# logicxin/SwiftMPI

Hardware: AMD Instinct MI355X
Metric: SGNS trained words/sec at 1/8 GPUs; sparse push/pull HBM GB/s vs peak (higher is better)
Workload: dtype f32 table, block-fp intermediates (int32 mantissas/row exponent), f64 accumulate; 1 GPU; word2vec CBOW-NS (the reference's 'SGNS' app) text8-shaped corpus 17005207 tokens, vocab 253628, dim 300, window 5, negative 5, sample 1e-05, minibatch 5000 lines of 1000 tokens, table in one HBM shard; global_batch=5000, parallelism=1 GPU, one HBM shard, batches_per_epoch=5

## Files before the change

### swiftmpi_amd/csrc/swps_w2v.hip

```cpp
#include <algorithm>
#include <cstdlib>
#include <cstdio>

#include "swps_w2v_ctx.h"

using namespace swps;

namespace {

__global__ void k_vid_keys(const int32_t *__restrict__ K, uint64_t n, const uint64_t *__restrict__ vkeys,
                           uint64_t *__restrict__ out) {
  uint64_t i = (uint64_t)blockIdx.x * blockDim.x + threadIdx.x;
  if (i < n) out[i] = vkeys[K[i]];
}

__global__ void k_stamp_rows(const uint32_t *__restrict__ rows, uint64_t n, uint32_t cap, uint32_t stamp,
                             uint32_t *__restrict__ mark) {
  const uint64_t i = (uint64_t)blockIdx.x * blockDim.x + threadIdx.x;
  if (i < n && rows[i] < cap) mark[rows[i]] = stamp;
}
__global__ void k_flag_rows(const uint32_t *__restrict__ rows, uint64_t n, uint32_t cap, uint32_t stamp,
                            const uint32_t *__restrict__ mark, uint8_t *__restrict__ flags) {
  const uint64_t i = (uint64_t)blockIdx.x * blockDim.x + threadIdx.x;
  if (i < n) flags[i] = rows[i] >= cap || mark[rows[i]] == stamp;
// ... 7 lines not shown
  if (!t || !cfg || !out) return fail(SWPS_E_CFG, "null argument");
  *out = nullptr;
  if (t->cfg.layout != SWPS_LAYOUT_W2V) return fail(SWPS_E_CFG, "table layout must be SWPS_LAYOUT_W2V");
  SWPS_TRY(check_app_table(t));
  SWPS_HIP(hipSetDevice(t->cfg.device));
  swps_w2v *w = new swps_w2v();
  w->t = t;
  w->cfg = *cfg;
  w->D = t->cfg.dim;
  w->W = cfg->window;
  w->N = cfg->negative;
  w->f64 = t->cfg.dtype == SWPS_F64;
  w->s = t->stream;
  w->timer.on = cfg->profile != 0;
  if (const char *e = getenv("SWPS_XCD_ORDER")) w->xcd_order = atoi(e) != 0;
  if (const char *e = getenv("SWPS_PUSH_T")) w->push_t = atoi(e) != 0;
  if (const char *e = getenv("SWPS_FUSED_PUSH")) w->fused_push = atoi(e) != 0;
  if (const char *e = getenv("SWPS_COMBINE")) w->combine = atoi(e);
  if (const char *e = getenv("SWPS_COMBINE_MIN")) w->combine_min = strtoull(e, nullptr, 10);
  if (const char *e = getenv("SWPS_FULL_LINES")) w->full_lines = atoi(e) != 0;
  if (const char *e = getenv("SWPS_SPLIT_PUSH")) w->split_push = atoi(e);
  if (const char *e = getenv("SWPS_SPLIT_GRADS")) w->split_grads = atoi(e) != 0;
  if (const char *e = getenv("SWPS_PUSH_GRID")) w->push_grid = (uint32_t)std::max(0, atoi(e));
  if (const char *e = getenv("SWPS_MULTI_SORT")) w->multi_sort = atoi(e);
  if (const char *e = getenv("SWPS_MULTI_CHUNK")) w->multi_chunk = (uint32_t)std::min(128, std::max(0, atoi(e)));
  if (const char *e = getenv("SWPS_MULTI_SORT_MIN")) w->multi_sort_min = strtoull(e, nullptr, 10);
  if (const char *e = getenv("SWPS_ROW_PAD")) w->row_pad = atoi(e) != 0;
  if (const char *e = getenv("SWPS_UNI_INDEX")) w->uni_index = atoi(e) != 0;
  if (const char *e = getenv("SWPS_SEG4")) w->seg4 = atoi(e) != 0;
  if (const char *e = getenv("SWPS_TOK_LOCAL")) w->tok_local = atoi(e) != 0;
  if (const char *e = getenv("SWPS_ITEM_HEADS")) w->item_heads = atoi(e) != 0;
  if (const char *e = getenv("SWPS_CACHE_PAD")) w->cache_pad = atoi(e) != 0;
  if (const char *e = getenv("SWPS_OVERLAP")) w->overlap = atoi(e);
  if (const char *e = getenv("SWPS_REC_GENERIC")) w->rec_generic = atoi(e) != 0;
  if (const char *e = getenv("SWPS_GATHER_GRID")) w->gather_grid = std::max(64, atoi(e));
  if (const char *e = getenv("SWPS_PUSH_WPE")) w->push_wpe = atoi(e);
  if (const char *e = getenv("SWPS_PUSH_UNR8")) w->push_unr = atoi(e) ? 8 : 4;
  int rc = check_cfg(w);
  if (!rc && hipHostMalloc((void **)&w->h_small, 64) != hipSuccess) rc = fail(SWPS_E_OOM, "pinned alloc");
  if (!rc) rc = w->d_rows_touched.ensure(16);
  if (!rc && hipMemset(w->d_rows_touched.p, 0, 16) != hipSuccess) rc = fail(SWPS_E_HIP, "memset");
  if (!rc) rc = w->d_gstats.ensure(32);
  if (!rc && hipMemset(w->d_gstats.p, 0, 32) != hipSuccess) rc = fail(SWPS_E_HIP, "memset");
  if (!rc) rc = upload_lcg_constants();
  if (rc) {
    if (w->h_small) (void)hipHostFree(w->h_small);
    delete w;
    return rc;
  }
  *out = w;
  return SWPS_OK;
}

int swps_w2v_destroy(swps_w2v *w) {
  if (!w) return SWPS_OK;
  (void)hipSetDevice(w->t->cfg.device);
  (void)hipStreamSynchronize(w->s);
  if (w->s_prep) {
    (void)hipStreamSynchronize(w->s_prep);
    (void)hipStreamDestroy(w->s_prep);
  }
  if (w->s_side) {
    (void)hipStreamSynchronize(w->s_side);
    (void)hipStreamDestroy(w->s_side);
  }
  if (w->ev_learn) (void)hipEventDestroy(w->ev_learn);
  if (w->ev_prep) (void)hipEventDestroy(w->ev_prep);
  if (w->ev_fwd) (void)hipEventDestroy(w->ev_fwd);
  if (w->ev_half) (void)hipEventDestroy(w->ev_half);
  if (w->ev_gat) (void)hipEventDestroy(w->ev_gat);
  if (w->h_small) (void)hipHostFree(w->h_small);
  delete w->drv;
  delete w;
  (void)hipGetLastError();
  return SWPS_OK;
}

int swps_w2v_load_text(swps_w2v *w, const char *path) {
  if (!w->cfg.minibatch_vocab && !w->cfg.host_ingest) {
    FILE *f = fopen(path, "rb");
    if (!f) return fail(SWPS_E_IO, std::string("no such file or directory: ") + path);
    std::vector<char> text;
    char chunk[1 << 16];
    size_t k;
    while ((k = fread(chunk, 1, sizeof(chunk), f)) > 0) text.insert(text.end(), chunk, chunk + k);
    fclose(f);
    if (!memchr(text.data(), 0, text.size())) {
      SWPS_HIP(hipSetDevice(w->t->cfg.device));
      DevMem d_keys;
      uint64_t nt = 0;
      std::vector<int64_t> off;
      SWPS_TRY(tokenize_gpu(w, text, d_keys, nt, off));
      std::vector<char>().swap(text);
      SWPS_TRY(ingest_gpu(w, d_keys, nt, std::move(off)));
      SWPS_TRY(schedule_gpu(w));
      return upload_corpus(w);
    }
  }
  FILE *f = fopen(path, "rb");
  if (!f) return fail(SWPS_E_IO, std::string("no such file or directory: ") + path);
// ... 123 lines not shown
}

int swps_w2v_train_batches(swps_w2v *w, uint64_t count) {
  if (!w->inited) return fail(SWPS_E_STATE, "call swps_w2v_init first");
  if (w->drv) {
    SWPS_HIP(hipSetDevice(w->t->cfg.device));
    return w->drv->steps(count);
  }
  if (w->sharded) return fail(SWPS_E_STATE, "sharded context: drive it with request / serve_pull / step / serve_push");
  SWPS_HIP(hipSetDevice(w->t->cfg.device));
  const bool ov = w->overlap > 0 || (w->overlap < 0 && w->max_tok <= kOverlapTok);
  if (ov && count > 1 && !w->cfg.minibatch_vocab && w->trace.size() >= w->trace_cap && !w->pb.valid)
    return train_overlapped(w, count);
  for (uint64_t i = 0; i < count; i++) SWPS_TRY(learn_step(w));
  return SWPS_OK;
}

int swps_w2v_train_epochs(swps_w2v *w, int32_t niters) {
  if (w->drv) {
    if (w->drv->spe && w->drv->cursor % w->drv->spe) return fail(SWPS_E_STATE, "not at an epoch boundary");
    SWPS_TRY(swps_w2v_train_batches(w, (uint64_t)niters * w->drv->spe));
    return swps_w2v_sync(w);
  }
  if (w->cursor % std::max<size_t>(1, w->batches.size()) != 0) return fail(SWPS_E_STATE, "not at an epoch boundary");
  SWPS_TRY(swps_w2v_train_batches(w, (uint64_t)niters * w->batches.size()));
  return swps_w2v_sync(w);
}

int swps_w2v_sync(swps_w2v *w) {
  SWPS_HIP(hipSetDevice(w->t->cfg.device));
  if (w->drv) SWPS_TRY(w->drv->sync());
  SWPS_HIP(hipStreamSynchronize(w->s));
  if (w->ss) SWPS_HIP(hipStreamSynchronize(w->ss));
  w->timer.resolve();
  return SWPS_OK;
}

int swps_w2v_stats(swps_w2v *w, uint64_t *o) {
  o[0] = w->st_batches;
  o[1] = w->st_kept;
  o[2] = w->st_words;
  o[3] = w->st_pairs;
  o[4] = w->lstate;
  o[5] = w->fstate;
  o[6] = w->st_pulled;
  o[7] = w->st_pushed;
  uint64_t rt[2] = {0, 0};
  SWPS_HIP(hipStreamSynchronize(w->s));
  SWPS_HIP(hipMemcpy(rt, w->d_rows_touched.p, 16, hipMemcpyDeviceToHost));
  o[8] = rt[0];
  o[9] = rt[1];
  return SWPS_OK;
}

int swps_w2v_gather_stats(swps_w2v *w, uint64_t *out2) {
  SWPS_HIP(hipStreamSynchronize(w->s));
  SWPS_HIP(hipMemcpy(out2, w->d_gstats.p, 16, hipMemcpyDeviceToHost));
  return SWPS_OK;
}

int swps_w2v_sum_stats(swps_w2v *w, uint64_t *out8) {
  SWPS_HIP(hipStreamSynchronize(w->s));
  SWPS_HIP(hipMemcpy(out8, w->d_gstats.p, 32, hipMemcpyDeviceToHost));
  out8[4] = w->st_fused;
  out8[5] = w->st_sums;
  out8[6] = w->st_fused_g;
// ... 420 lines not shown
  if (head[1] != w2v_corpus_fp(w) || head[2] != V || head[3] != ((uint64_t)w->D | ((uint64_t)es << 32)))
    return fail(SWPS_E_CFG, "snapshot was taken on a different corpus");
  if (head[4] != w->t->snap_sum)
    return fail(SWPS_E_STATE, "the table was not restored from the table snapshot saved with this worker state "
                              "(swps_restore <prefix>.table of the same save first)");
  std::vector<char> ch(V * w->D * es), cv(ch.size());
  SWPS_TRY(f.get(ch.data(), ch.size()));
  SWPS_TRY(f.get(cv.data(), cv.size()));
  SWPS_TRY(f.finish_read());
  if (!w->sharded) {
    DevMem dk;
    SWPS_TRY(upload(dk, w->vocab_keys, w->s));
    SWPS_TRY(table_lookup(w->t, dk.as<uint64_t>(), V, w->d_vid_row.as<uint32_t>(), w->s));
    if (table_check_error(w->t, w->s) != SWPS_OK)
      return fail(SWPS_E_STATE, "the table lacks the worker's vocab rows: swps_restore its table snapshot first");
  }
  if (!ch.empty()) {
    SWPS_HIP(hipMemcpy2D(w->d_cache_h.p, (size_t)w->cs * es, ch.data(), w->D * es, w->D * es, V,
                         hipMemcpyHostToDevice));
    SWPS_HIP(hipMemcpy2D(w->d_cache_v.p, (size_t)w->cs * es, cv.data(), w->D * es, w->D * es, V,
                         hipMemcpyHostToDevice));
  }
  SWPS_HIP(hipMemcpy(w->d_rows_touched.p, st + 9, 16, hipMemcpyHostToDevice));
  w->cursor = st[0];
  w->lstate = st[1];
  w->fstate = st[2];
  w->st_batches = st[3];
  w->st_kept = st[4];
  w->st_words = st[5];
  w->st_pairs = st[6];
  w->st_pulled = st[7];
  w->st_pushed = st[8];
  w->pb = swps_w2v::Prepped();
  const uint64_t nb = std::max<uint64_t>(1, w->batches.size());
  if (w->cursor % nb != 0) SWPS_TRY(plan_epoch(w));
  if (w->drv) {
    if (w->cursor % nb != 0) return fail(SWPS_E_STATE, "library-driven sharded state not at an epoch boundary");
    w->drv->cursor = w->cursor / nb * w->drv->spe;
    if (w->drv->ops.set_serve_stream) SWPS_TRY(w->drv->ops.set_serve_stream(w, w->drv->S));
  }
  w->inited = true;
  return SWPS_OK;
}

}
```

### swiftmpi_amd/csrc/swps_w2v_ctx.h

```cpp
#pragma once
#include <limits>
#include <memory>
#include <utility>
#include <vector>

#include "swps_internal.h"

namespace swps {

constexpr int32_t kTabRow = 0x40000000;
constexpr int kUShift = 10;

constexpr int kBfpMaxD = 512;
inline int bfp_ld(int D, int RB) { return (D + RB * D / 4 + 1 + 31) / 32 * 32; }
inline int bfp_shape(int D) {
  const int nch = D / 256, rem = D % 256;
  if (rem == 0) return 10 * nch;
  if (rem <= 128) return 10 * nch + (rem + 63) / 64;
  return 10 * (nch + 1);
}

enum { KT_KEEP = 0, KT_FWD, KT_SORT, KT_GATHER, KT_PUSH, KT_PULL, KT_REC, KT_N };

inline int row_ld(int D, size_t es, bool pad = true) {
// ... 142 lines not shown
  std::vector<uint64_t> icounts;
  std::vector<int32_t> init_order;
  DevMem d_vkeys, d_init_order, d_serve_rows, d_push_rows;
  DevMem d_mark;
  const uint32_t *pull_rows = nullptr;
  struct Parts {
    const void *vals[2] = {nullptr, nullptr};
    const uint32_t *pos[2] = {nullptr, nullptr};
    uint64_t n[2] = {0, 0};
  } parts;
  uint32_t mark_stamp = 0;
  hipStream_t ss = nullptr;
  int64_t slot = -1;
  struct SlotRows {
    DevMem rows, sorted;
    uint64_t n = 0;
    bool sorted_valid = false;
  };
  std::vector<std::unique_ptr<SlotRows>> slot_rows;
  std::vector<uint32_t> plan_P;
  std::vector<int32_t> allUK;
  std::vector<uint64_t> bstarts;
  std::vector<int32_t> bcnt_tok;
  uint64_t gather_end = 0;
  DevMem d_bstarts, d_UK, d_bcnt_tok, d_tw;
  std::vector<uint2> alias;
  DevMem d_alias;
  struct Prepped {
    bool valid = false, records = false, sorted = false, msorted = false;
    uint64_t bi = 0, P = 0, nt = 0, HOFF = 0, M = 0, max_items = 0;
    uint32_t U = 0;
  } pb;
  static constexpr int kPrepBufs = 15;
  DevMem alt[kPrepBufs];
  bool alt_local_ready = false;
  int overlap = -1;
  hipStream_t s_prep = nullptr;
  hipEvent_t ev_learn = nullptr, ev_prep = nullptr;
  hipEvent_t fwd_event = nullptr;
  DevMem *prep_set[kPrepBufs] = {&d_pos_tok, &d_rec,  &d_pkeys, &d_pvals, &d_pkeys_s, &d_pvals_s, &d_tmp,
                                 &d_seg,     &d_icnt, &d_ioff,  &d_desc,  &d_lead,    &d_multi, &d_krow, &d_local};
  uint64_t st_batches = 0, st_kept = 0, st_words = 0, st_pairs = 0, st_pulled = 0, st_pushed = 0;
  uint64_t st_sums = 0, st_fused = 0, st_fused_g = 0, st_split = 0;
  uint64_t trace_cap = 0;
  std::vector<int64_t> trace;
  Timer timer;
};

namespace swps {

constexpr uint32_t kChunk = 128;
inline uint32_t multi_chunk(const swps_w2v *w, uint64_t) { return w->multi_chunk ? w->multi_chunk : kChunk; }
constexpr uint64_t kOverlapTok = 1000000;

int check_cfg(swps_w2v *w);
int ingest(swps_w2v *w, const std::vector<uint64_t> &tok_keys, std::vector<int64_t> &&line_off);
void unigram_starts(const uint64_t *keys, const int32_t *counts, size_t V, uint64_t T, std::vector<uint64_t> &starts);
void build_schedule(swps_w2v *w);
int build_schedule_mb(swps_w2v *w);
int tokenize_gpu(swps_w2v *w, const std::vector<char> &text, DevMem &d_keys, uint64_t &nt,
                 std::vector<int64_t> &line_off);
int token_keys_gpu(swps_w2v *w, const uint32_t *word_ids, uint64_t ntok, const uint64_t *word_keys, uint64_t nwords,
                   DevMem &d_keys);
int ingest_gpu(swps_w2v *w, DevMem &d_keys, uint64_t nt, std::vector<int64_t> &&line_off);
int schedule_gpu(swps_w2v *w);
int upload_corpus(swps_w2v *w);

int upload_lcg_constants();
int plan_epoch(swps_w2v *w);
int prep_batch(swps_w2v *w);

int learn_step(swps_w2v *w, const void *d_vals = nullptr, void *d_grads = nullptr);
int train_overlapped(swps_w2v *w, uint64_t count);
int pull_all(swps_w2v *w);
int rand_init_gpu(swps_w2v *w);
int set_hv(swps_w2v *w, const double *hv);
int install_init(swps_w2v *w, const void *d_vals);

}
```

### swiftmpi_amd/csrc/swps_w2v_ingest.hip

```cpp
#include <algorithm>
#include <cmath>
#include <map>
#include <unordered_map>
#include <unordered_set>

#include "swps_scan.h"
#include "swps_sort.h"
#include "swps_w2v_ctx.h"

using namespace swps;

namespace {

__global__ void k_build_unigram(const uint64_t *__restrict__ starts, uint32_t V, uint64_t T, int32_t *__restrict__ table) {
  uint64_t a = (uint64_t)blockIdx.x * blockDim.x + threadIdx.x;
  uint64_t stride = (uint64_t)gridDim.x * blockDim.x;
  for (; a < T; a += stride) {
    uint32_t lo = 0, hi = V;
    while (hi - lo > 1) {
      uint32_t mid = (lo + hi) >> 1;
      if (starts[mid] <= a)
        lo = mid;
      else
        hi = mid;
// ... 710 lines not shown
  SWPS_TRY(lix.ensure((nb + 1) * 4));
  k_text_flags<<<nblk(nb + 1), 256, 0, s>>>(d_text.as<char>(), nb, st.as<uint32_t>(), nlf.as<uint32_t>());
  SWPS_HIP(hipGetLastError());
  SWPS_TRY(exclusive_scan(st.as<const uint32_t>(), tix.as<uint32_t>(), nb + 1, tmp, s));
  SWPS_TRY(exclusive_scan(nlf.as<const uint32_t>(), lix.as<uint32_t>(), nb + 1, tmp, s));
  uint32_t tot[2];
  SWPS_HIP(hipMemcpyAsync(&tot[0], tix.as<uint32_t>() + nb, 4, hipMemcpyDeviceToHost, s));
  SWPS_HIP(hipMemcpyAsync(&tot[1], lix.as<uint32_t>() + nb, 4, hipMemcpyDeviceToHost, s));
  SWPS_HIP(hipStreamSynchronize(s));
  nt = tot[0];
  const uint64_t nnl = tot[1];
  const uint64_t nlines = nnl + ((nb && text[nb - 1] != '\n') ? 1 : 0);
  SWPS_TRY(tstart.ensure(std::max<uint64_t>(nt, 1) * 8));
  SWPS_TRY(d_off.ensure((nlines + 2) * 8));
  SWPS_HIP(hipMemsetAsync(d_off.p, 0, 8, s));
  if (nb)
    k_text_index<<<nblk(nb), 256, 0, s>>>(d_text.as<char>(), nb, st.as<uint32_t>(), tix.as<uint32_t>(),
                                           lix.as<uint32_t>(), tstart.as<uint64_t>(), d_off.as<int64_t>());
  SWPS_HIP(hipGetLastError());
  SWPS_TRY(d_keys.ensure(std::max<uint64_t>(nt, 1) * 8));
  if (nt)
    k_text_keys<<<nblk(nt), 256, 0, s>>>(d_text.as<char>(), nb, tstart.as<uint64_t>(), nt,
                                          w->cfg.key_mode == SWPS_KEY_ATOI, d_keys.as<uint64_t>());
  SWPS_HIP(hipGetLastError());
  line_off.assign(nlines + 1, 0);
  if (nnl) SWPS_HIP(hipMemcpyAsync(line_off.data(), d_off.p, (nnl + 1) * 8, hipMemcpyDeviceToHost, s));
  SWPS_HIP(hipStreamSynchronize(s));
  line_off[nlines] = (int64_t)nt;
  return SWPS_OK;
}

int upload_corpus(swps_w2v *w) {
  hipStream_t s = w->s;
  const uint64_t V = w->vocab_keys.size();
  if (!w->tok_on_device) {
    SWPS_TRY(upload(w->d_tok, w->tok, s));
    SWPS_TRY(upload(w->d_tok_line, w->tok_line, s));
    SWPS_TRY(upload(w->d_K, w->allK, s));
  }
  SWPS_TRY(upload(w->d_line_off, w->line_off, s));
  SWPS_TRY(tok_fingerprint(w));
  std::vector<int64_t> btok;
  for (auto &b : w->batches) btok.push_back(w->line_off[b.l0]);
  btok.push_back(w->line_off[w->batches.back().l1]);
  SWPS_TRY(upload(w->d_btok, btok, s));
  std::vector<float> ran(V);
  for (uint64_t i = 0; i < V; i++) {
    float freq = float(w->counts[i]) / (float)w->train_words;
    ran[i] = (float)(1 - std::sqrt((double)(w->cfg.sample / freq)));
  }
  SWPS_TRY(upload(w->d_ran, ran, s));
  std::vector<float> ex(1000);
  for (int i = 0; i < 1000; i++) {
    float x = (i / (float)1000 * 2 - 1) * 6;
    float e = (float)std::exp((double)x);
    ex[i] = e / (e + 1);
  }
  SWPS_TRY(upload(w->d_exptab, ex, s));
  if (w->cfg.sampler == SWPS_SAMPLER_ALIAS) {
    if (!w->cfg.minibatch_vocab) {
      w->alias.clear();
      build_alias(w->counts.data(), V, w->alias);
    }
    SWPS_TRY(upload(w->d_alias, w->alias, s));
  }
  if (w->cfg.minibatch_vocab) {
    SWPS_TRY(upload(w->d_bstarts, w->bstarts, s));
    SWPS_TRY(upload(w->d_UK, w->allUK, s));
    SWPS_TRY(upload(w->d_bcnt_tok, w->bcnt_tok, s));
    SWPS_TRY(w->d_tw.ensure(w->batches.size() * 4));
  } else if (w->cfg.sampler != SWPS_SAMPLER_ALIAS) {
    std::vector<uint64_t> starts;
    unigram_starts(w->vocab_keys.data(), w->counts.data(), V, w->cfg.unigram_size, starts);
    SWPS_TRY(upload(w->d_starts, starts, s));
    SWPS_TRY(w->d_unigram.ensure(w->cfg.unigram_size * 4));
    k_build_unigram<<<4096, 256, 0, s>>>(w->d_starts.as<uint64_t>(), (uint32_t)V, w->cfg.unigram_size,
                                         w->d_unigram.as<int32_t>());
    SWPS_HIP(hipGetLastError());
    const uint64_t nb1 = ((w->cfg.unigram_size - 1) >> kUShift) + 2;
    SWPS_TRY(w->d_uidx.ensure(nb1 * 4));
    k_build_uidx<<<nblk(nb1), 256, 0, s>>>(w->d_starts.as<uint64_t>(), (uint32_t)V, kUShift, nb1,
                                           w->d_uidx.as<int32_t>());
    SWPS_HIP(hipGetLastError());
  }
  const size_t es = w->f64 ? 8 : 4;
  w->cs = row_ld(w->D, es, w->cache_pad);
  SWPS_TRY(w->d_cache_h.ensure(V * w->cs * es));
  SWPS_TRY(w->d_cache_v.ensure(V * w->cs * es));
  SWPS_TRY(w->d_local.ensure(V * 4));
  SWPS_HIP(hipMemsetAsync(w->d_local.p, 0xFF, V * 4, s));
  SWPS_TRY(w->d_vid_row.ensure(V * 4));
  SWPS_HIP(hipStreamSynchronize(s));
  return SWPS_OK;
}

}
```

### swiftmpi_amd/csrc/swps_w2v_learn.hip

```cpp
#include <hip/hip_ext.h>

#include <algorithm>
#include <type_traits>

#include "swps_rand.h"
#include "swps_w2v_ctx.h"
#include "swps_wave.h"

using namespace swps;

namespace {

template <typename T> struct V16;
template <> struct V16<float> {
  using V = float4;
  static constexpr int E = 4;
};
template <> struct V16<double> {
  using V = double2;
  static constexpr int E = 2;
};


template <typename T>
// ... 1392 lines not shown
  if (pb.records) SWPS_TRY((forward<T, A>(w, pb)));
  if (w->fwd_event) SWPS_HIP(hipEventRecord(w->fwd_event, s));
  const SumPlan pl = sum_plan<T, A>(w, pb, d_grads != nullptr);
  hipStream_t gs = s;
  if (pl.split) {
    if (!w->s_side) {
      int lo = 0, hi = 0;
      SWPS_HIP(hipDeviceGetStreamPriorityRange(&lo, &hi));
      SWPS_HIP(hipStreamCreateWithPriority(&w->s_side, hipStreamNonBlocking, hi));
      SWPS_HIP(hipEventCreateWithFlags(&w->ev_fwd, hipEventDisableTiming));
      SWPS_HIP(hipEventCreateWithFlags(&w->ev_gat, hipEventDisableTiming));
    }
    SWPS_HIP(hipEventRecord(w->ev_fwd, s));
    SWPS_HIP(hipStreamWaitEvent(w->s_side, w->ev_fwd, 0));
    gs = w->s_side;
  }
  if (pb.sorted) SWPS_TRY((gradient_sums<T, A>(w, pb, pl, gs)));
  if (U > 0) SWPS_TRY((push<T, A>(w, pb, pl, K, d_vals, d_grads)));
  w->pb.valid = false;
  w->cursor++;
  return SWPS_OK;
}

}

namespace swps {

int learn_step(swps_w2v *w, const void *d_vals, void *d_grads) {
  if (w->f64) return learn_batch<double, double>(w, d_vals, (double *)d_grads);
  if (inter64(w->cfg)) return learn_batch<float, double>(w, d_vals, (double *)d_grads);
  return learn_batch<float, float>(w, d_vals, (float *)d_grads);
}

static void swap_prep_set(swps_w2v *w) {
  for (int k = 0; k < swps_w2v::kPrepBufs; k++) {
    std::swap(w->prep_set[k]->p, w->alt[k].p);
    std::swap(w->prep_set[k]->bytes, w->alt[k].bytes);
  }
}

int train_overlapped(swps_w2v *w, uint64_t count) {
  if (!w->s_prep) {
    int lo = 0, hi = 0;
    SWPS_HIP(hipDeviceGetStreamPriorityRange(&lo, &hi));
    const char *pe = getenv("SWPS_PREP_PRIO");
    if (pe && atoi(pe) == 0)
      SWPS_HIP(hipStreamCreateWithFlags(&w->s_prep, hipStreamNonBlocking));
    else if (pe && atoi(pe) == 1)
      SWPS_HIP(hipStreamCreateWithPriority(&w->s_prep, hipStreamNonBlocking, lo));
    else
      SWPS_HIP(hipStreamCreateWithPriority(&w->s_prep, hipStreamNonBlocking, hi));
    SWPS_HIP(hipEventCreateWithFlags(&w->ev_learn, hipEventDisableTiming));
    SWPS_HIP(hipEventCreateWithFlags(&w->ev_prep, hipEventDisableTiming));
  }
  const uint64_t V = w->vocab_keys.size();
  if (!w->alt_local_ready) {
    DevMem &al = w->alt[swps_w2v::kPrepBufs - 1];
    SWPS_TRY(al.ensure(V * 4));
    SWPS_HIP(hipMemsetAsync(al.p, 0xFF, V * 4, w->s));
    w->alt_local_ready = true;
  }
  const hipStream_t s = w->s;
  bool prep_pending = false;
  if (w->overlap == 2) {
    for (uint64_t i = 0; i < count; i++) {
      if (!w->pb.valid) SWPS_TRY(prep_batch(w));
      if (prep_pending) SWPS_HIP(hipStreamWaitEvent(s, w->ev_prep, 0));
      w->fwd_event = i + 1 < count ? w->ev_learn : nullptr;
      const int lrc = learn_step(w);
      w->fwd_event = nullptr;
      SWPS_TRY(lrc);
      prep_pending = false;
      if (i + 1 < count) {
        SWPS_HIP(hipStreamWaitEvent(w->s_prep, w->ev_learn, 0));
        swap_prep_set(w);
        w->s = w->s_prep;
        w->pb = swps_w2v::Prepped();
        const int rc = prep_batch(w);
        w->s = s;
        SWPS_TRY(rc);
        SWPS_HIP(hipEventRecord(w->ev_prep, w->s_prep));
        prep_pending = true;
      }
    }
    if (prep_pending) SWPS_HIP(hipStreamWaitEvent(s, w->ev_prep, 0));
    return SWPS_OK;
  }
  for (uint64_t i = 0; i < count; i++) {
    if (!w->pb.valid) SWPS_TRY(prep_batch(w));
    const swps_w2v::Prepped cur = w->pb;
    swps_w2v::Prepped next;
    if (i + 1 < count) {
      SWPS_HIP(hipEventRecord(w->ev_learn, s));
      SWPS_HIP(hipStreamWaitEvent(w->s_prep, w->ev_learn, 0));
      swap_prep_set(w);
      w->s = w->s_prep;
      w->cursor++;
      w->pb = swps_w2v::Prepped();
      const int rc = prep_batch(w);
      next = w->pb;
      w->cursor--;
      w->s = s;
      swap_prep_set(w);
      SWPS_TRY(rc);
    }
    if (prep_pending) SWPS_HIP(hipStreamWaitEvent(s, w->ev_prep, 0));
    if (i + 1 < count) SWPS_HIP(hipEventRecord(w->ev_prep, w->s_prep));
    prep_pending = i + 1 < count;
    w->pb = cur;
    SWPS_TRY(learn_step(w));
    if (prep_pending) {
      swap_prep_set(w);
      w->pb = next;
    }
  }
  return SWPS_OK;
}

template <typename T> static int pull_all_t(swps_w2v *w) {
  const uint64_t V = w->vocab_keys.size();
  k_pull<T><<<nblk(V * 64), 256, 0, w->s>>>(nullptr, (uint32_t)V, w->d_vid_row.as<uint32_t>(), w->t->rows.as<T>(),
                                            w->D, w->d_cache_h.as<T>(), w->d_cache_v.as<T>(), w->d_local.as<int32_t>(),
                                            0, w->cs);
  SWPS_HIP(hipGetLastError());
  SWPS_HIP(hipStreamSynchronize(w->s));
  return SWPS_OK;
}
int pull_all(swps_w2v *w) { return w->f64 ? pull_all_t<double>(w) : pull_all_t<float>(w); }

template <typename T> static int rand_init_t(swps_w2v *w) {
  const uint64_t V = w->vocab_keys.size();
  const int D = w->D;
  const std::vector<uint32_t> base = glibc_base(w->cfg.rand_seed);
  const uint64_t total = V * 2 * (uint64_t)D;
  const uint64_t first = 344 + w->cfg.rand_offset;
  DevMem d_base;
  SWPS_TRY(upload(d_base, base, w->s));
  const uint64_t nthr = (total + kRandRun - 1) / kRandRun;
  if (total) {
    k_rand_init<T><<<nblk(nthr, 64), 64, 0, w->s>>>(d_base.as<uint32_t>(), first, total, D,
                                                    w->d_vid_row.as<uint32_t>(), w->t->rows.as<T>());
    k_zero_sums<T><<<nblk(total), 256, 0, w->s>>>(w->d_vid_row.as<uint32_t>(), V, D, w->t->rows.as<T>());
  }
  SWPS_HIP(hipGetLastError());
  SWPS_HIP(hipStreamSynchronize(w->s));
  return pull_all_t<T>(w);
}
// ... 30 lines not shown
```

### swiftmpi_amd/csrc/swps_w2v_prep.hip

```cpp
#include <algorithm>

#include "swps_scan.h"
#include "swps_sort.h"
#include "swps_w2v_ctx.h"

using namespace swps;

namespace {

__device__ __forceinline__ int32_t unigram_lookup(const uint64_t *__restrict__ starts, const int32_t *__restrict__ idx,
                                                  int shift, uint32_t V, uint64_t slot) {
  const uint64_t b = slot >> shift;
  uint32_t lo = (uint32_t)idx[b], hi = min((uint32_t)idx[b + 1] + 1u, V);
  while (hi - lo > 1) {
    const uint32_t mid = (lo + hi) >> 1;
    if (starts[mid] <= slot)
      lo = mid;
    else
      hi = mid;
  }
  return (int32_t)lo;
}

constexpr int kKeepRun = 16;
// ... 586 lines not shown
  SWPS_TRY(w->d_neu1.ensure(maxP * nrow));
  SWPS_TRY(w->d_neu1e.ensure(maxP * nrow));
  SWPS_TRY(w->d_pg.ensure(HOFF * 4));
  const uint64_t U = w->max_U;
  if (U) {
    int bits = 1;
    while ((1ULL << bits) <= U) bits++;
    for (uint64_t n : {M, std::min<uint64_t>(M, kSmallSort - 1)}) {
      SWPS_TRY(sort_pairs(w->d_tmp, w->d_pkeys.as<uint32_t>(), w->d_pkeys_s.as<uint32_t>(), w->d_pvals.as<uint32_t>(),
                          w->d_pvals_s.as<uint32_t>(), n, bits, w->s, false));
      SWPS_TRY(sort_pairs_iota(w->d_tmp, w->d_pkeys.as<uint32_t>(), w->d_pkeys_s.as<uint32_t>(),
                               w->d_pvals_s.as<uint32_t>(), n, bits, w->s, false));
    }
    const uint64_t max_items = 2ULL * U + M / multi_chunk(w, maxP) + 1;
    SWPS_TRY(w->d_lead.ensure((max_items / 8 + 2) * 4));
    SWPS_TRY(w->d_seg.ensure(U * 16));
    SWPS_TRY(w->d_icnt.ensure((2ULL * U + 1) * 4));
    SWPS_TRY(w->d_ioff.ensure((2ULL * U + 1) * 4));
    SWPS_TRY(w->d_desc.ensure(max_items * 16));
    SWPS_TRY(w->d_partial.ensure(max_items * D * a));
    SWPS_TRY(w->d_multi.ensure((max_items + 1) * 4));
    if (w->multi_sort && maxP >= w->multi_sort_min) {
      SWPS_TRY(w->d_pkeys.ensure(max_items * 4));
      SWPS_TRY(w->d_pvals.ensure(max_items * 4));
      SWPS_TRY(w->d_icnt.ensure(max_items * 4));
      for (uint64_t n : {max_items, std::min<uint64_t>(max_items, kSmallSort - 1)})
        SWPS_TRY(sort_pairs(w->d_tmp, w->d_pkeys.as<uint32_t>(), w->d_icnt.as<uint32_t>(), w->d_pvals.as<uint32_t>(),
                            w->d_multi.as<uint32_t>(), n, 16, w->s, false));
    }
  }
  return SWPS_OK;
}

int plan_epoch(swps_w2v *w) {
  hipStream_t s = w->s;
  const uint64_t nb = w->batches.size();
  const uint64_t L = w->batches[nb - 1].l1;
  const uint64_t T = (uint64_t)w->line_off[L];
  const bool sample_on = w->cfg.sample >= 0;
  SWPS_TRY(w->d_kflag.ensure((T + 1) * 4));
  SWPS_TRY(w->d_kscan.ensure((T + 1) * 4));
  SWPS_TRY(w->d_ldraw.ensure((L + 1) * 8));
  SWPS_TRY(w->d_ldoff.ensure((L + 1) * 8));
  hipEvent_t ek = w->timer.begin(s);
  std::vector<int32_t> tw;
  if (w->cfg.minibatch_vocab) {
    const uint64_t e = w->cursor / nb;
    uint64_t per_epoch = w->gather_end;
    for (auto &b : w->batches) per_epoch += b.gathered;
    uint64_t acc = w->train_words + e * per_epoch;
    tw.resize(nb);
    for (uint64_t b = 0; b < nb; b++) {
      acc += w->batches[b].gathered;
      tw[b] = (int32_t)(uint32_t)acc;
    }
    SWPS_HIP(hipMemcpyAsync(w->d_tw.p, tw.data(), nb * 4, hipMemcpyHostToDevice, s));
    k_keep_mb<<<nblk((T + kKeepRun) / kKeepRun), 256, 0, s>>>(w->d_bcnt_tok.as<int32_t>(), T, w->d_btok.as<int64_t>(),
                                                              (uint32_t)nb, w->d_tw.as<int32_t>(), w->cfg.sample,
                                                              w->fstate, sample_on, w->d_kflag.as<int32_t>());
  } else {
    k_keep<<<nblk((T + 64 * kKeepIt) / (64 * kKeepIt) * 64), 256, 0, s>>>(w->d_tok.as<int32_t>(), T, w->d_ran.as<float>(),
                                                                          w->fstate, sample_on, w->d_kflag.as<int32_t>());
  }
  SWPS_HIP(hipGetLastError());
  SWPS_TRY(exclusive_scan(w->d_kflag.as<int32_t>(), w->d_kscan.as<int32_t>(), T + 1, w->d_tmp, s));
  k_line_draws<<<nblk(L + 1), 256, 0, s>>>(w->d_line_off.as<int64_t>(), L, w->d_kscan.as<int32_t>(), w->N,
                                           w->d_ldraw.as<uint64_t>());
  SWPS_HIP(hipGetLastError());
  SWPS_TRY(exclusive_scan(w->d_ldraw.as<uint64_t>(), w->d_ldoff.as<uint64_t>(), L + 1, w->d_tmp, s));
  w->timer.end(KT_KEEP, ek, s);
  SWPS_TRY(w->d_bounds.ensure((nb + 1) * 4));
  k_bounds<<<nblk(nb + 1), 256, 0, s>>>(w->d_kscan.as<int32_t>(), w->d_btok.as<int64_t>(), nb + 1,
                                        w->d_bounds.as<int32_t>());
  SWPS_HIP(hipGetLastError());
  std::vector<int32_t> ks(nb + 1);
  SWPS_HIP(hipMemcpyAsync(ks.data(), w->d_bounds.p, (nb + 1) * 4, hipMemcpyDeviceToHost, s));
  uint64_t draws = 0;
  SWPS_HIP(hipMemcpyAsync(&draws, w->d_ldoff.as<uint64_t>() + L, 8, hipMemcpyDeviceToHost, s));
  SWPS_HIP(hipStreamSynchronize(s));
  w->plan_P.resize(nb);
  uint64_t maxP = 0;
  for (uint64_t i = 0; i < nb; i++) {
    w->plan_P[i] = (uint32_t)(ks[i + 1] - ks[i]);
    maxP = std::max<uint64_t>(maxP, w->plan_P[i]);
  }
  SWPS_TRY(presize(w, maxP));
  w->lstate_epoch = w->lstate;
  w->fstate_epoch = w->fstate;
  w->lstate = lcg_jump(w->lstate, draws, kLcgA, kLcgC);
  if (sample_on) w->fstate = lcg_jump(w->fstate, T, kFlcgA, kLcgC);
  return SWPS_OK;
}


int prep_batch(swps_w2v *w) {
  if (w->pb.valid) return SWPS_OK;
  const uint64_t nb = w->batches.size();
  if (w->cursor % nb == 0) SWPS_TRY(plan_epoch(w));
  const uint64_t bi = w->cursor % nb;
  const swps_w2v::Batch &B = w->batches[bi];
  hipStream_t s = w->s;
  Timer &tm = w->timer;
  const int W = w->W, N = w->N;
  const uint64_t t0 = (uint64_t)w->line_off[B.l0], t1 = (uint64_t)w->line_off[B.l1];
  const uint64_t nt = t1 - t0;
  const uint32_t U = B.U;
  const int32_t *K = w->d_K.as<int32_t>() + B.kofs;
  const uint64_t P = w->plan_P[bi];
  auto &pb = w->pb;
  pb = swps_w2v::Prepped();
  pb.bi = bi;
  pb.P = P;
  pb.U = U;
  pb.nt = nt;
  const bool tracing = w->trace.size() < w->trace_cap;
  const bool recs = P > 0 && (U > 0 || tracing);
  if (recs) SWPS_TRY(w->d_pos_tok.ensure(P * 4));
  const bool will_sort = recs && U > 0;
  if (will_sort) {
    SWPS_TRY(w->d_seg.ensure((uint64_t)U * 16));
    const uint64_t mi = 2ULL * U + P * (uint64_t)(N + 1 + 2 * W) / multi_chunk(w, P) + 1;
    SWPS_TRY(w->d_lead.ensure((mi / 8 + 2) * 4));
    SWPS_TRY(w->d_multi.ensure((mi + 1) * 4));
  }
  const bool krow = U > 0 && !w->sharded && (w->bfp || (w->tail && w->fused_push));
  if (krow) SWPS_TRY(w->d_krow.ensure((uint64_t)U * 4));
  if (U || recs) {
    k_batch_setup<<<nblk(std::max<uint64_t>(U, recs ? nt : 0)), 256, 0, s>>>(
        K, U, w->d_local.as<int32_t>(), w->d_kscan.as<int32_t>(), t0, recs ? nt : 0,
        recs ? w->d_pos_tok.as<int32_t>() : nullptr, will_sort ? w->d_seg.as<uint4>() : nullptr,
        will_sort ? w->d_lead.as<uint32_t>() : nullptr, will_sort ? w->d_multi.as<uint32_t>() : nullptr,
// ... 129 lines not shown
```

Before: 454.4 million words/s.

## Deepen batch prep pipeline to multiple buffer sets and plan next epoch ahead

Generalizes the double-buffered prep overlap into a ring of up to three prep buffer sets, so prep can run one or two batches ahead of learning on the side stream. Epoch planning (keep flags, scans, bounds) is now launched ahead on the prep stream into alternate buffers with pinned host readback, which removes the blocking stream sync at each epoch boundary. The cost is extra device memory for additional buffer sets and more complex event and state bookkeeping, including dropping the lookahead plan whenever the RNG state changes.

```diff
diff --git a/swiftmpi_amd/csrc/swps_w2v.hip b/swiftmpi_amd/csrc/swps_w2v.hip
--- a/swiftmpi_amd/csrc/swps_w2v.hip
+++ b/swiftmpi_amd/csrc/swps_w2v.hip
@@ -63,6 +63,8 @@
   if (const char *e = getenv("SWPS_ITEM_HEADS")) w->item_heads = atoi(e) != 0;
   if (const char *e = getenv("SWPS_CACHE_PAD")) w->cache_pad = atoi(e) != 0;
   if (const char *e = getenv("SWPS_OVERLAP")) w->overlap = atoi(e);
+  if (const char *e = getenv("SWPS_PREP_AHEAD")) w->prep_ahead = std::min(2, std::max(0, atoi(e)));
+  if (const char *e = getenv("SWPS_PLAN_AHEAD")) w->plan_ahead = atoi(e) != 0;
   if (const char *e = getenv("SWPS_REC_GENERIC")) w->rec_generic = atoi(e) != 0;
   if (const char *e = getenv("SWPS_GATHER_GRID")) w->gather_grid = std::max(64, atoi(e));
   if (const char *e = getenv("SWPS_PUSH_WPE")) w->push_wpe = atoi(e);
@@ -95,8 +97,13 @@
     (void)hipStreamSynchronize(w->s_side);
     (void)hipStreamDestroy(w->s_side);
   }
-  if (w->ev_learn) (void)hipEventDestroy(w->ev_learn);
-  if (w->ev_prep) (void)hipEventDestroy(w->ev_prep);
+  for (hipEvent_t e : w->ev_set_learn)
+    if (e) (void)hipEventDestroy(e);
+  for (hipEvent_t e : w->ev_set_prep)
+    if (e) (void)hipEventDestroy(e);
+  for (hipEvent_t e : {w->ev_pfwd, w->ev_entry, w->ev_plan})
+    if (e) (void)hipEventDestroy(e);
+  if (w->h_plan) (void)hipHostFree(w->h_plan);
   if (w->ev_fwd) (void)hipEventDestroy(w->ev_fwd);
   if (w->ev_half) (void)hipEventDestroy(w->ev_half);
   if (w->ev_gat) (void)hipEventDestroy(w->ev_gat);
@@ -286,6 +293,7 @@
   if (w->drv) SWPS_TRY(w->drv->sync());
   SWPS_HIP(hipStreamSynchronize(w->s));
   if (w->ss) SWPS_HIP(hipStreamSynchronize(w->ss));
+  if (w->s_prep) SWPS_HIP(hipStreamSynchronize(w->s_prep));
   w->timer.resolve();
   return SWPS_OK;
 }
@@ -772,6 +780,7 @@
   w->st_pulled = st[7];
   w->st_pushed = st[8];
   w->pb = swps_w2v::Prepped();
+  plan_drop_ahead(w);
   const uint64_t nb = std::max<uint64_t>(1, w->batches.size());
   if (w->cursor % nb != 0) SWPS_TRY(plan_epoch(w));
   if (w->drv) {
diff --git a/swiftmpi_amd/csrc/swps_w2v_ctx.h b/swiftmpi_amd/csrc/swps_w2v_ctx.h
--- a/swiftmpi_amd/csrc/swps_w2v_ctx.h
+++ b/swiftmpi_amd/csrc/swps_w2v_ctx.h
@@ -198,14 +198,29 @@
     uint32_t U = 0;
   } pb;
   static constexpr int kPrepBufs = 15;
-  DevMem alt[kPrepBufs];
-  bool alt_local_ready = false;
+  static constexpr int kPrepSets = 3;
+  DevMem alt[kPrepSets][kPrepBufs];
+  int set_cur = 0;
+  bool set_ready[kPrepSets] = {};
   int overlap = -1;
+  int prep_ahead = 0;
+  int plan_ahead = 1;
   hipStream_t s_prep = nullptr;
-  hipEvent_t ev_learn = nullptr, ev_prep = nullptr;
+  hipEvent_t ev_set_learn[kPrepSets] = {}, ev_set_prep[kPrepSets] = {};
+  hipEvent_t ev_pfwd = nullptr, ev_entry = nullptr;
   hipEvent_t fwd_event = nullptr;
   DevMem *prep_set[kPrepBufs] = {&d_pos_tok, &d_rec,  &d_pkeys, &d_pvals, &d_pkeys_s, &d_pvals_s, &d_tmp,
                                  &d_seg,     &d_icnt, &d_ioff,  &d_desc,  &d_lead,    &d_multi, &d_krow, &d_local};
+  struct PlanAhead {
+    bool valid = false;
+    uint64_t lstate_in = 0, fstate_in = 0;
+  } ahead;
+  static constexpr int kPlanBufs = 5;
+  DevMem plan_alt[kPlanBufs], d_plan_tmp;
+  DevMem *plan_set[kPlanBufs] = {&d_kflag, &d_kscan, &d_ldraw, &d_ldoff, &d_bounds};
+  hipEvent_t ev_plan = nullptr;
+  int32_t *h_plan = nullptr;
+  uint64_t h_plan_nb = 0;
   uint64_t st_batches = 0, st_kept = 0, st_words = 0, st_pairs = 0, st_pulled = 0, st_pushed = 0;
   uint64_t st_sums = 0, st_fused = 0, st_fused_g = 0, st_split = 0;
   uint64_t trace_cap = 0;
@@ -235,6 +250,10 @@
 int upload_lcg_constants();
 int plan_epoch(swps_w2v *w);
 int prep_batch(swps_w2v *w);
+void use_prep_set(swps_w2v *w, int k);
+int presize_sets(swps_w2v *w, int nsets);
+int plan_issue_ahead(swps_w2v *w);
+void plan_drop_ahead(swps_w2v *w);
 
 int learn_step(swps_w2v *w, const void *d_vals = nullptr, void *d_grads = nullptr);
 int train_overlapped(swps_w2v *w, uint64_t count);
diff --git a/swiftmpi_amd/csrc/swps_w2v_ingest.hip b/swiftmpi_amd/csrc/swps_w2v_ingest.hip
--- a/swiftmpi_amd/csrc/swps_w2v_ingest.hip
+++ b/swiftmpi_amd/csrc/swps_w2v_ingest.hip
@@ -766,6 +766,7 @@
 
 int upload_corpus(swps_w2v *w) {
   hipStream_t s = w->s;
+  plan_drop_ahead(w);
   const uint64_t V = w->vocab_keys.size();
   if (!w->tok_on_device) {
     SWPS_TRY(upload(w->d_tok, w->tok, s));
@@ -823,6 +824,7 @@
   SWPS_TRY(w->d_cache_v.ensure(V * w->cs * es));
   SWPS_TRY(w->d_local.ensure(V * 4));
   SWPS_HIP(hipMemsetAsync(w->d_local.p, 0xFF, V * 4, s));
+  for (int k = 0; k < swps_w2v::kPrepSets; k++) w->set_ready[k] = k == w->set_cur;
   SWPS_TRY(w->d_vid_row.ensure(V * 4));
   SWPS_HIP(hipStreamSynchronize(s));
   return SWPS_OK;
diff --git a/swiftmpi_amd/csrc/swps_w2v_learn.hip b/swiftmpi_amd/csrc/swps_w2v_learn.hip
--- a/swiftmpi_amd/csrc/swps_w2v_learn.hip
+++ b/swiftmpi_amd/csrc/swps_w2v_learn.hip
@@ -1448,14 +1448,9 @@
   return learn_batch<float, float>(w, d_vals, (float *)d_grads);
 }
 
-static void swap_prep_set(swps_w2v *w) {
-  for (int k = 0; k < swps_w2v::kPrepBufs; k++) {
-    std::swap(w->prep_set[k]->p, w->alt[k].p);
-    std::swap(w->prep_set[k]->bytes, w->alt[k].bytes);
-  }
-}
-
 int train_overlapped(swps_w2v *w, uint64_t count) {
+  constexpr int kSets = swps_w2v::kPrepSets;
+  const bool large = w->max_tok > kOverlapTok;
   if (!w->s_prep) {
     int lo = 0, hi = 0;
     SWPS_HIP(hipDeviceGetStreamPriorityRange(&lo, &hi));
@@ -1466,69 +1461,69 @@
       SWPS_HIP(hipStreamCreateWithPriority(&w->s_prep, hipStreamNonBlocking, lo));
     else
       SWPS_HIP(hipStreamCreateWithPriority(&w->s_prep, hipStreamNonBlocking, hi));
-    SWPS_HIP(hipEventCreateWithFlags(&w->ev_learn, hipEventDisableTiming));
-    SWPS_HIP(hipEventCreateWithFlags(&w->ev_prep, hipEventDisableTiming));
-  }
+    for (int k = 0; k < kSets; k++) {
+      SWPS_HIP(hipEventCreateWithFlags(&w->ev_set_learn[k], hipEventDisableTiming));
+      SWPS_HIP(hipEventCreateWithFlags(&w->ev_set_prep[k], hipEventDisableTiming));
+    }
+    SWPS_HIP(hipEventCreateWithFlags(&w->ev_pfwd, hipEventDisableTiming));
+    SWPS_HIP(hipEventCreateWithFlags(&w->ev_entry, hipEventDisableTiming));
+  }
+  const hipStream_t s = w->s;
+  const int A = w->prep_ahead ? w->prep_ahead : large ? 2 : 1, NS = A + 1;
+  const bool after_fwd = w->overlap == 2;
   const uint64_t V = w->vocab_keys.size();
-  if (!w->alt_local_ready) {
-    DevMem &al = w->alt[swps_w2v::kPrepBufs - 1];
-    SWPS_TRY(al.ensure(V * 4));
-    SWPS_HIP(hipMemsetAsync(al.p, 0xFF, V * 4, w->s));
-    w->alt_local_ready = true;
-  }
-  const hipStream_t s = w->s;
-  bool prep_pending = false;
-  if (w->overlap == 2) {
-    for (uint64_t i = 0; i < count; i++) {
-      if (!w->pb.valid) SWPS_TRY(prep_batch(w));
-      if (prep_pending) SWPS_HIP(hipStreamWaitEvent(s, w->ev_prep, 0));
-      w->fwd_event = i + 1 < count ? w->ev_learn : nullptr;
-      const int lrc = learn_step(w);
-      w->fwd_event = nullptr;
-      SWPS_TRY(lrc);
-      prep_pending = false;
-      if (i + 1 < count) {
-        SWPS_HIP(hipStreamWaitEvent(w->s_prep, w->ev_learn, 0));
-        swap_prep_set(w);
-        w->s = w->s_prep;
-        w->pb = swps_w2v::Prepped();
-        const int rc = prep_batch(w);
-        w->s = s;
-        SWPS_TRY(rc);
-        SWPS_HIP(hipEventRecord(w->ev_prep, w->s_prep));
-        prep_pending = true;
-      }
-    }
-    if (prep_pending) SWPS_HIP(hipStreamWaitEvent(s, w->ev_prep, 0));
+  for (int k = 0; k < NS; k++)
+    if (!w->set_ready[k]) {
+      DevMem &al = w->alt[k][swps_w2v::kPrepBufs - 1];
+      SWPS_TRY(al.ensure(V * 4));
+      SWPS_HIP(hipMemsetAsync(al.p, 0xFF, V * 4, s));
+      w->set_ready[k] = true;
+    }
+  SWPS_TRY(presize_sets(w, NS));
+  const uint64_t c0 = w->cursor;
+  const int first = w->set_cur;
+  auto set_of = [&](uint64_t j) { return (int)((first + j) % NS); };
+  swps_w2v::Prepped q[kSets];
+  bool learned[kSets] = {};
+  auto issue_prep = [&](uint64_t j, hipEvent_t gate) -> int {
+    const int k = set_of(j), kc = w->set_cur;
+    const uint64_t cur = w->cursor;
+    if (gate) SWPS_HIP(hipStreamWaitEvent(w->s_prep, gate, 0));
+    use_prep_set(w, k);
+    w->s = w->s_prep;
+    w->cursor = c0 + j;
+    w->pb = swps_w2v::Prepped();
+    int rc = prep_batch(w);
+    if (rc == SWPS_OK) rc = plan_issue_ahead(w);
+    q[k] = w->pb;
+    w->pb = swps_w2v::Prepped();
+    w->cursor = cur;
+    w->s = s;
+    use_prep_set(w, kc);
+    SWPS_TRY(rc);
+    SWPS_HIP(hipEventRecord(w->ev_set_prep[k], w->s_prep));
     return SWPS_OK;
-  }
+  };
+  SWPS_TRY(prep_batch(w));
+  q[first] = w->pb;
+  SWPS_HIP(hipEventRecord(w->ev_entry, s));
+  SWPS_HIP(hipStreamWaitEvent(w->s_prep, w->ev_entry, 0));
+  SWPS_TRY(plan_issue_ahead(w));
+  for (uint64_t j = 1; j < (uint64_t)A && j < count; j++) SWPS_TRY(issue_prep(j, nullptr));
   for (uint64_t i = 0; i < count; i++) {
-    if (!w->pb.valid) SWPS_TRY(prep_batch(w));
-    const swps_w2v::Prepped cur = w->pb;
-    swps_w2v::Prepped next;
-    if (i + 1 < count) {
-      SWPS_HIP(hipEventRecord(w->ev_learn, s));
-      SWPS_HIP(hipStreamWaitEvent(w->s_prep, w->ev_learn, 0));
-      swap_prep_set(w);
-      w->s = w->s_prep;
-      w->cursor++;
-      w->pb = swps_w2v::Prepped();
-      const int rc = prep_batch(w);
-      next = w->pb;
-      w->cursor--;
-      w->s = s;
-      swap_prep_set(w);
-      SWPS_TRY(rc);
-    }
-    if (prep_pending) SWPS_HIP(hipStreamWaitEvent(s, w->ev_prep, 0));
-    if (i + 1 < count) SWPS_HIP(hipEventRecord(w->ev_prep, w->s_prep));
-    prep_pending = i + 1 < count;
-    w->pb = cur;
-    SWPS_TRY(learn_step(w));
-    if (prep_pending) {
-      swap_prep_set(w);
-      w->pb = next;
-    }
+    const uint64_t j = i + A;
+    const int k = set_of(i);
+    if (!after_fwd && j < count) SWPS_TRY(issue_prep(j, learned[set_of(j)] ? w->ev_set_learn[set_of(j)] : nullptr));
+    use_prep_set(w, k);
+    w->pb = q[k];
+    if (i > 0) SWPS_HIP(hipStreamWaitEvent(s, w->ev_set_prep[k], 0));
+    w->fwd_event = after_fwd && j < count ? w->ev_pfwd : nullptr;
+    const int rc = learn_step(w);
+    w->fwd_event = nullptr;
+    SWPS_TRY(rc);
+    SWPS_HIP(hipEventRecord(w->ev_set_learn[k], s));
+    learned[k] = true;
+    if (after_fwd && j < count) SWPS_TRY(issue_prep(j, w->ev_pfwd));
   }
   return SWPS_OK;
 }
diff --git a/swiftmpi_amd/csrc/swps_w2v_prep.hip b/swiftmpi_amd/csrc/swps_w2v_prep.hip
--- a/swiftmpi_amd/csrc/swps_w2v_prep.hip
+++ b/swiftmpi_amd/csrc/swps_w2v_prep.hip
@@ -642,16 +642,17 @@
   return SWPS_OK;
 }
 
-int plan_epoch(swps_w2v *w) {
-  hipStream_t s = w->s;
+static int plan_launch(swps_w2v *w, hipStream_t s, uint64_t fstate, DevMem *const ps[swps_w2v::kPlanBufs], DevMem &tmp,
+                       int32_t *ks, uint64_t *draws) {
+  DevMem &d_kflag = *ps[0], &d_kscan = *ps[1], &d_ldraw = *ps[2], &d_ldoff = *ps[3], &d_bounds = *ps[4];
   const uint64_t nb = w->batches.size();
   const uint64_t L = w->batches[nb - 1].l1;
   const uint64_t T = (uint64_t)w->line_off[L];
   const bool sample_on = w->cfg.sample >= 0;
-  SWPS_TRY(w->d_kflag.ensure((T + 1) * 4));
-  SWPS_TRY(w->d_kscan.ensure((T + 1) * 4));
-  SWPS_TRY(w->d_ldraw.ensure((L + 1) * 8));
-  SWPS_TRY(w->d_ldoff.ensure((L + 1) * 8));
+  SWPS_TRY(d_kflag.ensure((T + 1) * 4));
+  SWPS_TRY(d_kscan.ensure((T + 1) * 4));
+  SWPS_TRY(d_ldraw.ensure((L + 1) * 8));
+  SWPS_TRY(d_ldoff.ensure((L + 1) * 8));
   hipEvent_t ek = w->timer.begin(s);
   std::vector<int32_t> tw;
   if (w->cfg.minibatch_vocab) {
@@ -667,27 +668,29 @@
     SWPS_HIP(hipMemcpyAsync(w->d_tw.p, tw.data(), nb * 4, hipMemcpyHostToDevice, s));
     k_keep_mb<<<nblk((T + kKeepRun) / kKeepRun), 256, 0, s>>>(w->d_bcnt_tok.as<int32_t>(), T, w->d_btok.as<int64_t>(),
                                                               (uint32_t)nb, w->d_tw.as<int32_t>(), w->cfg.sample,
-                                                              w->fstate, sample_on, w->d_kflag.as<int32_t>());
+                                                              fstate, sample_on, d_kflag.as<int32_t>());
   } else {
     k_keep<<<nblk((T + 64 * kKeepIt) / (64 * kKeepIt) * 64), 256, 0, s>>>(w->d_tok.as<int32_t>(), T, w->d_ran.as<float>(),
-                                                                          w->fstate, sample_on, w->d_kflag.as<int32_t>());
+                                                                          fstate, sample_on, d_kflag.as<int32_t>());
   }
   SWPS_HIP(hipGetLastError());
-  SWPS_TRY(exclusive_scan(w->d_kflag.as<int32_t>(), w->d_kscan.as<int32_t>(), T + 1, w->d_tmp, s));
-  k_line_draws<<<nblk(L + 1), 256, 0, s>>>(w->d_line_off.as<int64_t>(), L, w->d_kscan.as<int32_t>(), w->N,
-                                           w->d_ldraw.as<uint64_t>());
+  SWPS_TRY(exclusive_scan(d_kflag.as<int32_t>(), d_kscan.as<int32_t>(), T + 1, tmp, s));
+  k_line_draws<<<nblk(L + 1), 256, 0, s>>>(w->d_line_off.as<int64_t>(), L, d_kscan.as<int32_t>(), w->N,
+                                           d_ldraw.as<uint64_t>());
   SWPS_HIP(hipGetLastError());
-  SWPS_TRY(exclusive_scan(w->d_ldraw.as<uint64_t>(), w->d_ldoff.as<uint64_t>(), L + 1, w->d_tmp, s));
+  SWPS_TRY(exclusive_scan(d_ldraw.as<uint64_t>(), d_ldoff.as<uint64_t>(), L + 1, tmp, s));
   w->timer.end(KT_KEEP, ek, s);
-  SWPS_TRY(w->d_bounds.ensure((nb + 1) * 4));
-  k_bounds<<<nblk(nb + 1), 256, 0, s>>>(w->d_kscan.as<int32_t>(), w->d_btok.as<int64_t>(), nb + 1,
-                                        w->d_bounds.as<int32_t>());
+  SWPS_TRY(d_bounds.ensure((nb + 1) * 4));
+  k_bounds<<<nblk(nb + 1), 256, 0, s>>>(d_kscan.as<int32_t>(), w->d_btok.as<int64_t>(), nb + 1, d_bounds.as<int32_t>());
   SWPS_HIP(hipGetLastError());
-  std::vector<int32_t> ks(nb + 1);
-  SWPS_HIP(hipMemcpyAsync(ks.data(), w->d_bounds.p, (nb + 1) * 4, hipMemcpyDeviceToHost, s));
-  uint64_t draws = 0;
-  SWPS_HIP(hipMemcpyAsync(&draws, w->d_ldoff.as<uint64_t>() + L, 8, hipMemcpyDeviceToHost, s));
-  SWPS_HIP(hipStreamSynchronize(s));
+  SWPS_HIP(hipMemcpyAsync(ks, d_bounds.p, (nb + 1) * 4, hipMemcpyDeviceToHost, s));
+  SWPS_HIP(hipMemcpyAsync(draws, d_ldoff.as<uint64_t>() + L, 8, hipMemcpyDeviceToHost, s));
+  return SWPS_OK;
+}
+
+static int plan_commit(swps_w2v *w, const int32_t *ks, uint64_t draws) {
+  const uint64_t nb = w->batches.size();
+  const uint64_t T = (uint64_t)w->line_off[w->batches[nb - 1].l1];
   w->plan_P.resize(nb);
   uint64_t maxP = 0;
   for (uint64_t i = 0; i < nb; i++) {
@@ -698,15 +701,90 @@
   w->lstate_epoch = w->lstate;
   w->fstate_epoch = w->fstate;
   w->lstate = lcg_jump(w->lstate, draws, kLcgA, kLcgC);
-  if (sample_on) w->fstate = lcg_jump(w->fstate, T, kFlcgA, kLcgC);
+  if (w->cfg.sample >= 0) w->fstate = lcg_jump(w->fstate, T, kFlcgA, kLcgC);
   return SWPS_OK;
+}
+
+int plan_epoch(swps_w2v *w) {
+  const uint64_t nb = w->batches.size();
+  std::vector<int32_t> ks(nb + 1);
+  uint64_t draws = 0;
+  SWPS_TRY(plan_launch(w, w->s, w->fstate, w->plan_set, w->d_tmp, ks.data(), &draws));
+  SWPS_HIP(hipStreamSynchronize(w->s));
+  return plan_commit(w, ks.data(), draws);
+}
+
+int plan_issue_ahead(swps_w2v *w) {
+  if (w->ahead.valid || !w->plan_ahead || !w->s_prep || w->cfg.minibatch_vocab) return SWPS_OK;
+  const uint64_t nb = w->batches.size();
+  if (!w->ev_plan) SWPS_HIP(hipEventCreateWithFlags(&w->ev_plan, hipEventDisableTiming));
+  if (w->h_plan_nb < nb) {
+    SWPS_HIP(hipStreamSynchronize(w->s_prep));
+    if (w->h_plan) SWPS_HIP(hipHostFree(w->h_plan));
+    w->h_plan = nullptr;
+    w->h_plan_nb = 0;
+    SWPS_HIP(hipHostMalloc((void **)&w->h_plan, (nb + 2) / 2 * 8 + 8));
+    w->h_plan_nb = nb;
+  }
+  DevMem *ps[swps_w2v::kPlanBufs];
+  for (int k = 0; k < swps_w2v::kPlanBufs; k++) ps[k] = &w->plan_alt[k];
+  uint64_t *draws = (uint64_t *)(w->h_plan + (nb + 2) / 2 * 2);
+  SWPS_TRY(plan_launch(w, w->s_prep, w->fstate, ps, w->d_plan_tmp, w->h_plan, draws));
+  SWPS_HIP(hipEventRecord(w->ev_plan, w->s_prep));
+  w->ahead.valid = true;
+  w->ahead.lstate_in = w->lstate;
+  w->ahead.fstate_in = w->fstate;
+  return SWPS_OK;
+}
+
+void plan_drop_ahead(swps_w2v *w) {
+  if (!w->ahead.valid) return;
+  (void)hipStreamSynchronize(w->s_prep);
+  w->ahead.valid = false;
+}
+
+static int plan_take(swps_w2v *w) {
+  const uint64_t nb = w->batches.size();
+  SWPS_HIP(hipEventSynchronize(w->ev_plan));
+  w->ahead.valid = false;
+  for (int k = 0; k < swps_w2v::kPlanBufs; k++) {
+    std::swap(w->plan_set[k]->p, w->plan_alt[k].p);
+    std::swap(w->plan_set[k]->bytes, w->plan_alt[k].bytes);
+  }
+  return plan_commit(w, w->h_plan, *(const uint64_t *)(w->h_plan + (nb + 2) / 2 * 2));
+}
+
+int presize_sets(swps_w2v *w, int nsets) {
+  uint64_t maxP = 0;
+  for (uint32_t p : w->plan_P) maxP = std::max<uint64_t>(maxP, p);
+  const int cur = w->set_cur;
+  int rc = SWPS_OK;
+  for (int k = 0; k < nsets && rc == SWPS_OK; k++) {
+    use_prep_set(w, k);
+    rc = presize(w, maxP);
+  }
+  use_prep_set(w, cur);
+  return rc;
+}
+
+void use_prep_set(swps_w2v *w, int k) {
+  if (k == w->set_cur) return;
+  for (int from : {w->set_cur, k})
+    for (int b = 0; b < swps_w2v::kPrepBufs; b++) {
+      std::swap(w->prep_set[b]->p, w->alt[from][b].p);
+      std::swap(w->prep_set[b]->bytes, w->alt[from][b].bytes);
+    }
+  w->set_cur = k;
 }
 
 
 int prep_batch(swps_w2v *w) {
   if (w->pb.valid) return SWPS_OK;
   const uint64_t nb = w->batches.size();
-  if (w->cursor % nb == 0) SWPS_TRY(plan_epoch(w));
+  if (w->cursor % nb == 0) {
+    if (w->ahead.valid && (w->ahead.lstate_in != w->lstate || w->ahead.fstate_in != w->fstate)) plan_drop_ahead(w);
+    SWPS_TRY(w->ahead.valid ? plan_take(w) : plan_epoch(w));
+  }
   const uint64_t bi = w->cursor % nb;
   const swps_w2v::Batch &B = w->batches[bi];
   hipStream_t s = w->s;
```

Result: no change. 453.9 million words/s (-0.1%).
